# XiandaGuo/OpenStereo

Measured on NVIDIA H100. Metric: stereo_pairs_per_sec_gwcnet_256x512_d192, higher is better.
Workload: dtype f32

## Files before the change

openstereo_b200/csrc/conv3d_tcs2.cu:

```cuda
#include "tc_common.cuh"

namespace osb {

struct Tcs2Params {
  const float* x;
  const void* w;
  const float* scale;
  const float* shift;
  const float* residual;
  float* y;
  int B, D, H, Cin;
  int act;
  float kappa;
  unsigned int* overflow;
  int out_ndhwc, res_ndhwc;
  int items, hblocks;
  int Wr, ctiles;
  int ystride;
};

template <int COUT, int KC, int W, int TILES, bool GW = false>
struct Tcs2Cfg {
  static_assert(!GW || W == 128, "general-width tiles are 128-column segments of one output row");
  static constexpr int HALO = GW ? 1 : 0;
  static constexpr int CSTEP = 128 - HALO;
  static constexpr int R = 128 / W;
  static constexpr int ROWB = KC * 4;
  static constexpr int UNIT_BYTES = 128 * ROWB;
  static constexpr int N3 = 3 * COUT;
  static constexpr int G = 32;
  static constexpr int NG = COUT / G;
  static constexpr int B_SLICE = N3 * ROWB;
  static constexpr int B_SUB = 3 * G * ROWB;
  static constexpr int LD = 3 * G + 4;
  static constexpr int NLW = 5;
  static constexpr int FIXED_SMEM = 1024 + TC_BSLOTS * 3 * B_SUB + 128 * LD * 4 + 1024 + 2 * 4 * 2 * 32 * 4 + 3 * COUT * 4;
  static constexpr int STAGES = (232448 - FIXED_SMEM) / UNIT_BYTES < 10 ? (232448 - FIXED_SMEM) / UNIT_BYTES : 10;
  static_assert(STAGES >= NLW, "the ring must hold at least one unit per loader warp");
  static constexpr int NU = TILES * 3 * 2;
  static constexpr int HBLK = TILES * R;
  static constexpr int KSTEPS = KC / 16;
  static constexpr int LO = KC / 8;
  static constexpr int A_OFF = 0;
  static constexpr int B_OFF = A_OFF + STAGES * UNIT_BYTES;
  static constexpr int STAGE_OFF = B_OFF + TC_BSLOTS * 3 * B_SUB;
  static constexpr int BAR_OFF = STAGE_OFF + 128 * LD * 4;
  static constexpr int THREADS = 128 + 128 + 64;
  static constexpr size_t SMEM = 1024 + (size_t)BAR_OFF + 1024 + 2 * 4 * 2 * 32 * 4 + 3 * COUT * 4;
  static_assert(SMEM <= 232448, "shared memory budget of one CTA exceeded");
  static_assert(TILES == 1, "the consumer warpgroup holds one accumulator tile");
  static_assert(COUT % G == 0, "output channels come in groups of 32");
  static_assert(B_SUB % 1024 == 0 && UNIT_BYTES % 1024 == 0, "operand tiles must stay 1024-byte aligned");
};

template <int COUT, int KC, int W, int TILES, bool GW = false>
__global__ void __launch_bounds__(Tcs2Cfg<COUT, KC, W, TILES, GW>::THREADS, 1) conv3d_tcs2_kernel(const Tcs2Params p) {
  using C = Tcs2Cfg<COUT, KC, W, TILES, GW>;
  extern __shared__ __align__(1024) uint8_t smem_raw[];
  uint8_t* smem = reinterpret_cast<uint8_t*>((reinterpret_cast<uintptr_t>(smem_raw) + 1023) & ~static_cast<uintptr_t>(1023));
  uint8_t* a_buf = smem + C::A_OFF;
  uint8_t* b_buf = smem + C::B_OFF;
  float* stage = reinterpret_cast<float*>(smem + C::STAGE_OFF);
  uint64_t* bars = reinterpret_cast<uint64_t*>(smem + C::BAR_OFF);
  uint64_t* a_ready = bars;
  uint64_t* a_empty = a_ready + C::STAGES;
  uint64_t* b_full = a_empty + C::STAGES;
  uint64_t* b_empty = b_full + TC_BSLOTS * 3;
  float* xchg = reinterpret_cast<float*>(smem + C::BAR_OFF + 1024);
  float* s_scale = xchg + 2 * 4 * 2 * 32;
  float* s_shift = s_scale + COUT;
  float* zeros = s_shift + COUT;

  const int warp = threadIdx.x >> 5, lane = threadIdx.x & 31;
  const int nchunk = p.Cin / KC;
  const int Wp = GW ? p.Wr : W;
  const int YS = (W < 32 && p.ystride) ? p.ystride : COUT;
  const int ctiles = GW ? p.ctiles : 1;

  if (threadIdx.x == 0) {
    for (int s = 0; s < C::STAGES; ++s) {
      mbar_init(&a_ready[s], 32);
      mbar_init(&a_empty[s], 4);
    }
    for (int k = 0; k < TC_BSLOTS * 3; ++k) {
      mbar_init(&b_full[k], 1);
      mbar_init(&b_empty[k], 4);
    }
    fence_mbar_init();
  }
  for (int c = threadIdx.x; c < COUT; c += blockDim.x) {
    s_scale[c] = p.scale ? p.scale[c] : 1.f;
    s_shift[c] = p.shift ? p.shift[c] : 0.f;
    zeros[c] = 0.f;
  }
  __syncthreads();

  if (warp < 4) {
    const uint64_t dbase = (KC == 32) ? desc_sw128_base() : desc_sw64_base();
    constexpr uint32_t A_HALF = 64 * C::ROWB / 16;
    const uint32_t b16 = (smem_u32(b_buf) & 0x3FFFF) >> 4;
    const int Do = p.D / 2, Ho = p.H / 2;
    const int q = warp;
    const int m = q * 32 + lane;
    const int rr = m / W, wcol = m % W;
    const bool has_left_q = ((q * 32) % W) != 0;
    uint32_t unitc = 0, phc = 0, exc = 0;
    for (int it = blockIdx.x; it < p.items; it += gridDim.x) {
      const int cg = (it % C::NG) * C::G;
      const int it0 = it / C::NG;
      const int ct = it0 % ctiles;
      const int hb = (it0 / ctiles) % p.hblocks;
      const int d = (it0 / (ctiles * p.hblocks)) % Do;
      const int b = it0 / (ctiles * p.hblocks * Do);
      {
        float acc_e[2][C::G / 2], acc_o[2][C::G];
        uint32_t accum_e = 0, accum_o = 0;
        for (int kd = 0; kd < 3; ++kd) {
          const int din = 2 * d + kd - 1;
          if (din < 0 || din >= p.D) continue;
          for (int ch = 0; ch < nchunk; ++ch, ++phc) {
#pragma unroll
            for (int kh = 0; kh < 3; ++kh) {
              const uint32_t bslot = (phc & 1) * 3 + kh;
#pragma unroll
              for (int par = 0; par < 2; ++par) {
                const uint32_t slot = unitc % C::STAGES, ph = (unitc / C::STAGES) & 1;
                mbar_wait(&a_ready[slot], ph);
                if (par == 0) mbar_wait(&b_full[bslot], (phc >> 1) & 1);
                const uint64_t da0 = dbase | (uint64_t)((smem_u32(a_buf + slot * C::UNIT_BYTES) & 0x3FFFF) >> 4);
                const uint64_t db0 = dbase | (uint64_t)(b16 + (bslot * C::B_SUB + (par ? C::G * C::ROWB : 0)) / 16);
                wg_fence();
#pragma unroll
                for (int ks = 0; ks < C::KSTEPS; ++ks) {
                  if (par == 0) wg_mma_split<C::G>(acc_e, da0 + 2 * ks, A_HALF, db0 + 2 * ks, C::LO, ks > 0 ? 1u : accum_e);
                  else wg_mma_split<2 * C::G>(acc_o, da0 + 2 * ks, A_HALF, db0 + 2 * ks, C::LO, ks > 0 ? 1u : accum_o);
                }
                wg_commit();
                wg_wait_all();
                if (par == 0) accum_e = 1;
                else accum_o = 1;
                wg_release(&a_empty[slot], lane);
                if (par == 1) wg_release(&b_empty[bslot], lane);
                ++unitc;
              }
            }
          }
        }
        named_bar_sync(2, 128);
        wg_stage<C::G>(stage, C::LD, acc_e, warp, lane);
        wg_stage<2 * C::G>(stage + C::G, C::LD, acc_o, warp, lane);
        named_bar_sync(2, 128);
      }
      const int h0 = hb * C::HBLK;
      const int ntiles = min(TILES, (Ho - h0 + C::R - 1) / C::R);
      const int col = GW ? ct * C::CSTEP - C::HALO + m : wcol;
      const bool cvalid = !GW || (m >= C::HALO && col < Wp);
      const uint32_t vmask = GW ? __ballot_sync(0xffffffffu, cvalid) : 0xffffffffu;
      const float corr = 1.f + p.kappa * (float)(((d > 0) + 1 + (2 * d + 1 < p.D)) * nchunk * 3 * C::KSTEPS * 3);
      for (int t = 0; t < ntiles; ++t) {
        const int h = h0 + t * C::R + rr;
        const bool live = h < Ho;
        const ptrdiff_t vox = (((ptrdiff_t)b * Do + d) * Ho + h) * Wp + col;
        const size_t plane = (size_t)Do * Ho * Wp;
        const ptrdiff_t ncdhw0 = (ptrdiff_t)b * COUT * plane + ((ptrdiff_t)d * Ho + h) * Wp + col;
        {
          uint32_t raw[3][32];
#pragma unroll
          for (int kw = 0; kw < 3; ++kw)
#pragma unroll
            for (int c0 = 0; c0 < 32; c0 += 16) stage_ld16(stage + m * C::LD + kw * C::G + c0, &raw[kw][c0]);
          float* xb = xchg + (exc & 1) * (4 * 2 * 32);
          ++exc;
          if (lane == 31) {
#pragma unroll
            for (int i = 0; i < 32; ++i) xb[(q * 2) * 32 + i] = __uint_as_float(raw[1][i]);
          }
          named_bar_sync(1, 128);
          const float* xl = has_left_q ? xb + ((q - 1) * 2) * 32 : zeros;
          float out[32];
#pragma unroll
          for (int i0 = 0; i0 < 32; i0 += 4) {
            const float4 l4 = *reinterpret_cast<const float4*>(xl + i0);
            const float le[4] = {l4.x, l4.y, l4.z, l4.w};
#pragma unroll
            for (int k = 0; k < 4; ++k) {
              const int i = i0 + k;
              float left = __shfl_up_sync(0xffffffffu, __uint_as_float(raw[1][i]), 1);
              left = (lane == 0) ? le[k] : left;
              if (W < 32) left = (wcol == 0) ? 0.f : left;
              out[i] = ((left + __uint_as_float(raw[0][i])) + __uint_as_float(raw[2][i])) * corr;
            }
          }
          const uint32_t vm = (W < 32) ? __ballot_sync(0xffffffffu, live) : (live ? vmask : 0u);
          if (vm && p.out_ndhwc && (!p.residual || p.res_ndhwc)) {
            store_ndhwc_chunk32(stage + q * 32 * C::LD, lane, out, p.y + (vox - lane) * YS + cg,
                                p.residual ? p.residual + (vox - lane) * YS + cg : nullptr, YS, s_scale + cg, s_shift + cg, p.act,
                                vm);
          } else if (live && cvalid) {
#pragma unroll
            for (int i = 0; i < 32; ++i) out[i] = fmaf(out[i], s_scale[cg + i], s_shift[cg + i]);
            if (p.residual) {
              if (p.res_ndhwc) {
                const float4* rp = reinterpret_cast<const float4*>(p.residual + vox * YS + cg);
#pragma unroll
                for (int i = 0; i < 8; ++i) {
                  const float4 rv = __ldg(rp + i);
                  out[4 * i] += rv.x, out[4 * i + 1] += rv.y, out[4 * i + 2] += rv.z, out[4 * i + 3] += rv.w;
                }
              } else {
#pragma unroll
                for (int i = 0; i < 32; ++i) out[i] += __ldg(p.residual + ncdhw0 + (size_t)(cg + i) * plane);
              }
            }
            if (p.act == OSB_ACT_RELU) {
#pragma unroll
              for (int i = 0; i < 32; ++i) out[i] = fmaxf(out[i], 0.f);
            } else if (p.act == OSB_ACT_LEAKY) {
#pragma unroll
              for (int i = 0; i < 32; ++i) out[i] = out[i] > 0.f ? out[i] : 0.01f * out[i];
            }
            if (p.out_ndhwc) {
              float4* yp = reinterpret_cast<float4*>(p.y + vox * YS + cg);
#pragma unroll
              for (int i = 0; i < 8; ++i) yp[i] = make_float4(out[4 * i], out[4 * i + 1], out[4 * i + 2], out[4 * i + 3]);
            } else {
#pragma unroll
              for (int i = 0; i < 32; ++i) p.y[ncdhw0 + (size_t)(cg + i) * plane] = out[i];
            }
          }
        }
      }
    }
  }
  else if (warp < 8 || warp == 9) {
    const int lw = warp < 8 ? warp - 4 : 4;
    static_assert(KC == 16, "lane_voxel / unit-row mapping below is written for 64-byte operand rows");
    constexpr int CPR = KC / 4;
    constexpr int VPL = 32 / CPR;
    constexpr int NLD = 128 / VPL;
    static_assert(W % VPL == 0, "a load instruction must not straddle image rows");
    const int v0 = lane_voxel<KC>(lane), c = lane % CPR;
    float amax = 0.f;
    const int WI = 2 * Wp;
    const int Do = p.D / 2;
    uint32_t ubase = 0;
    int first = lw;
    auto fill = [&](const float* base, size_t rstride, size_t cstride, int h_first, int h_step, uint32_t u, int col0) {
      float4 v[NLD];
#pragma unroll
      for (int j = 0; j < NLD; ++j) {
        const int hin = h_first + h_step * ((VPL * j) / W);
        const size_t off = (size_t)((VPL * j) / W) * rstride + (size_t)((VPL * j) % W) * cstride;
        bool ok = hin >= 0 && hin < p.H;
        if (GW) ok = ok && (unsigned)(col0 + VPL * j) < (unsigned)Wp;
        v[j] = ok ? __ldg(reinterpret_cast<const float4*>(base + (ptrdiff_t)off)) : make_float4(0.f, 0.f, 0.f, 0.f);
      }
      const uint32_t slot = u % C::STAGES, ph = (u / C::STAGES) & 1;
      mbar_wait_relaxed(&a_empty[slot], ph ^ 1);
      uint8_t* tile = a_buf + slot * C::UNIT_BYTES;
#pragma unroll
      for (int j = 0; j < NLD; ++j) stage_f16_split<KC>(tile, v0 + VPL * j, c, v[j], amax);
      fence_proxy_async();
      mbar_arrive(&a_ready[slot]);
    };
    for (int it = blockIdx.x; it < p.items; it += gridDim.x) {
      const int it0 = it / C::NG;
      const int ct = it0 % ctiles;
      const int hb = (it0 / ctiles) % p.hblocks;
      const int od = (it0 / (ctiles * p.hblocks)) % Do;
      const int b = it0 / (ctiles * p.hblocks * Do);
      const int h0 = hb * C::HBLK;
      const int col0 = ct * C::CSTEP - C::HALO + v0;
      for (int kd = 0; kd < 3; ++kd) {
        const int din = 2 * od + kd - 1;
        if (din < 0 || din >= p.D) continue;
        const float* plane = p.x + ((size_t)b * p.D + din) * p.H * (size_t)WI * p.Cin;
        for (int ch = 0; ch < nchunk; ++ch) {
#pragma unroll 1
          for (int j = first; j < C::NU; j += C::NLW) {
            const int t = j / 6, kh = (j >> 1) % 3, par = j & 1;
            const int h_first = 2 * (h0 + t * C::R) + kh - 1;
            const float* base = plane + ((ptrdiff_t)h_first * WI + 2 * col0 + par) * p.Cin + ch * KC + c * 4;
            fill(base, (size_t)2 * WI * p.Cin, (size_t)2 * p.Cin, h_first, 2, ubase + j, col0);
          }
          ubase += C::NU;
          first = (first + C::NLW - C::NU % C::NLW) % C::NLW;
        }
      }
    }
    tc_report_overflow(p.overflow, amax);
  }
  else if (warp == 8) {
    if (elect_one()) {
      const uint8_t* wsrc = reinterpret_cast<const uint8_t*>(p.w);
      uint32_t phc = 0;
      for (int it = blockIdx.x; it < p.items; it += gridDim.x) {
        const int cg = (it % C::NG) * C::G;
        const int od = (it / C::NG / (ctiles * p.hblocks)) % (p.D / 2);
        for (int kd = 0; kd < 3; ++kd) {
          const int din = 2 * od + kd - 1;
          if (din < 0 || din >= p.D) continue;
          for (int ch = 0; ch < nchunk; ++ch, ++phc) {
            for (int kh = 0; kh < 3; ++kh) {
              const uint32_t slot = (phc & 1) * 3 + kh;
              const size_t slice = ((size_t)kd * nchunk + ch) * 3 + kh;
              mbar_wait_relaxed(&b_empty[slot], ((phc >> 1) & 1) ^ 1);
              mbar_arrive_expect_tx(&b_full[slot], C::B_SUB);
#pragma unroll
              for (int kw = 0; kw < 3; ++kw)
                bulk_g2s(b_buf + slot * C::B_SUB + kw * C::G * C::ROWB, wsrc + slice * C::B_SLICE + (size_t)(kw * COUT + cg) * C::ROWB,
                         C::G * C::ROWB, &b_full[slot]);
            }
          }
        }
      }
    }
    __syncwarp();
  }
}

template <int COUT, int KC, int W, int TILES, bool GW = false>
static int launch_tcs2(Tcs2Params& p, cudaStream_t stream) {
  using C = Tcs2Cfg<COUT, KC, W, TILES, GW>;
  auto kernel = conv3d_tcs2_kernel<COUT, KC, W, TILES, GW>;
  static PerDeviceFlag configured;
  if (!configured.here()) {
    cudaError_t e = cudaFuncSetAttribute(kernel, cudaFuncAttributeMaxDynamicSharedMemorySize, (int)C::SMEM);
    if (e != cudaSuccess) {
      set_error("conv3d_tcg: cannot reserve %zu bytes of shared memory: %s", C::SMEM, cudaGetErrorString(e));
      return OSB_ECUDA;
    }
    configured.here() = true;
  }
  if (W >= 32 && p.ystride && p.ystride != COUT) {
    set_error("conv3d_tcs2: channel slices are instantiated for W = 16 only");
    return OSB_EUNSUPPORTED;
  }
  p.hblocks = (p.H / 2 + C::HBLK - 1) / C::HBLK;
  if (GW) p.ctiles = (p.Wr + C::CSTEP - 1) / C::CSTEP;
  else p.Wr = W, p.ctiles = 1;
  const long long items = (long long)p.B * (p.D / 2) * p.hblocks * p.ctiles * C::NG;
  OSB_REQUIRE(items < (1ll << 31), "conv3d_tcs2: too many work items");
  p.items = (int)items;
  const int sms = sm_count();
  const int grid = (int)cap_persistent_grid(p.items < sms ? p.items : sms);
  static const std::string variant = tc_variant_name("tcs2<%d,%d,%d,%d,%d>", COUT, KC, W, TILES, (int)GW);
  set_tc_variant(variant.c_str());
  kernel<<<grid, C::THREADS, C::SMEM, stream>>>(p);
  count_launch();
  cudaError_t le = cudaGetLastError();
  if (le != cudaSuccess) {
    cudaFuncAttributes fa{};
    (void)cudaFuncGetAttributes(&fa, kernel);
    set_error("conv3d_tcs2_kernel<%d,%d,%d,%d>: launch failed: %s (threads %d, kernel maxThreadsPerBlock %d, regs %d, static smem %zu, "
              "dynamic smem %zu, max dynamic %d)", COUT, KC, W, TILES, cudaGetErrorString(le), C::THREADS, fa.maxThreadsPerBlock,
              fa.numRegs, fa.sharedSizeBytes, C::SMEM, fa.maxDynamicSharedSizeBytes);
    return OSB_ECUDA;
  }
  return OSB_OK;
}

}

extern "C" {

int osb_conv3d_s2_tc_supported(int Cin, int Cout, int D, int H, int W) {
  if (Cin % 16 != 0 || Cin < 16 || D % 2 || H % 2 || W % 2) return 0;
  if ((W == 128 && Cout == 64) || (W == 64 && (Cout == 64 || Cout == 96 || Cout == 128)) || (W == 32 && (Cout == 64 || Cout == 96)))
    return 1;
  return (osb_tc_general_width(W / 2) && (Cout == 64 || Cout == 128)) ? 1 : 0;
}

static int conv3d_k3_s2_tc_impl(const float* x_ndhwc, const void* w_split, const float* scale, const float* shift,
                                const float* residual, float* y, int B, int Cin, int Cout, int D, int H, int W, int act,
                                int out_ndhwc, int res_ndhwc, int ystride, osb_stream_t stream) {
  using namespace osb;
  OSB_REQUIRE(ystride == 0 || (ystride >= Cout && ystride % 4 == 0 && out_ndhwc && (!residual || res_ndhwc)),
              "conv3d_k3_s2_tc: a channel slice (ystride %d) needs channels-last tensors", ystride);
  OSB_REQUIRE(x_ndhwc && w_split && y, "conv3d_k3_s2_tc: null pointer");
  OSB_REQUIRE(B > 0 && D > 0 && H > 0, "conv3d_k3_s2_tc: empty shape");
  OSB_REQUIRE(osb_conv3d_s2_tc_supported(Cin, Cout, D, H, W), "conv3d_k3_s2_tc: unsupported shape Cin=%d Cout=%d D=%d H=%d W=%d", Cin,
              Cout, D, H, W);
  OSB_REQUIRE(act >= 0 && act <= 2, "conv3d_k3_s2_tc: unknown activation %d", act);
  Tcs2Params p{};
  p.x = x_ndhwc, p.w = w_split, p.scale = scale, p.shift = shift, p.residual = residual, p.y = y;
  p.B = B, p.D = D, p.H = H, p.Cin = Cin, p.act = act, p.out_ndhwc = out_ndhwc, p.res_ndhwc = res_ndhwc;
  p.kappa = rz_kappa(), p.overflow = tc_overflow_flag();
  p.ystride = ystride;
  OSB_REQUIRE(p.overflow, "tensor-core conv: cannot allocate the overflow flag");
  cudaStream_t s = (cudaStream_t)stream;
  if (W == 32 && Cout == 96) return launch_tcs2<96, 16, 16, 1>(p, s);
  if (W == 32 && Cout == 64) return launch_tcs2<64, 16, 16, 1>(p, s);
  if (W == 128 && Cout == 64) return launch_tcs2<64, 16, 64, 1>(p, s);
  if (W == 64 && Cout == 64) return launch_tcs2<64, 16, 32, 1>(p, s);
  if (W == 64 && Cout == 128) return launch_tcs2<128, 16, 32, 1>(p, s);
  if (W == 64 && Cout == 96) return launch_tcs2<96, 16, 32, 1>(p, s);
  p.Wr = W / 2;
  if (Cout == 64) return launch_tcs2<64, 16, 128, 1, true>(p, s);
  return launch_tcs2<128, 16, 128, 1, true>(p, s);
}

int osb_conv3d_k3_s2_tc_fwd(const float* x_ndhwc, const void* w_split, const float* scale, const float* shift,
                            const float* residual, float* y, int B, int Cin, int Cout, int D, int H, int W, int act,
                            int out_ndhwc, int res_ndhwc, osb_stream_t stream) {
  return conv3d_k3_s2_tc_impl(x_ndhwc, w_split, scale, shift, residual, y, B, Cin, Cout, D, H, W, act, out_ndhwc, res_ndhwc, 0, stream);
}

int osb_conv3d_k3_s2_tc_cs_fwd(const float* x_ndhwc, const void* w_split, const float* scale, const float* shift, float* y, int B,
                               int Cin, int Cout, int D, int H, int W, int act, int ystride, osb_stream_t stream) {
  return conv3d_k3_s2_tc_impl(x_ndhwc, w_split, scale, shift, nullptr, y, B, Cin, Cout, D, H, W, act, 1, 1, ystride, stream);
}
}
```

Measured before the change: 196.3.

## Share loaded input tiles across multiple consumer warpgroups in stride-2 conv3d

Lets several consumer warpgroups (TC_WGS) consume the same A-operand ring unit, each computing a different 32-channel output group, so the input tile is loaded once per item for several channel groups instead of once per group. The weight producer loads one B sub-tile per group into a wider slot, and warp registers are rebalanced with setmaxnreg. The epilogue stages accumulators in two 16-channel passes to fit per-warpgroup staging buffers. In exchange, shared memory per stage grows, fewer ring stages may fit, and warpgroups with no group to compute still have to wait and arrive on the barriers.

```diff
diff --git a/openstereo_b200/csrc/conv3d_tcs2.cu b/openstereo_b200/csrc/conv3d_tcs2.cu
--- a/openstereo_b200/csrc/conv3d_tcs2.cu
+++ b/openstereo_b200/csrc/conv3d_tcs2.cu
@@ -30,11 +30,16 @@
   static constexpr int N3 = 3 * COUT;
   static constexpr int G = 32;
   static constexpr int NG = COUT / G;
+  static constexpr int NP = (NG + TC_WGS - 1) / TC_WGS;
   static constexpr int B_SLICE = N3 * ROWB;
   static constexpr int B_SUB = 3 * G * ROWB;
-  static constexpr int LD = 3 * G + 4;
-  static constexpr int NLW = 5;
-  static constexpr int FIXED_SMEM = 1024 + TC_BSLOTS * 3 * B_SUB + 128 * LD * 4 + 1024 + 2 * 4 * 2 * 32 * 4 + 3 * COUT * 4;
+  static constexpr int B_SLOT = TC_WGS * B_SUB;
+  static constexpr int PC = 16;
+  static constexpr int NPASS = G / PC;
+  static constexpr int LD = 3 * PC + 4;
+  static constexpr int XCHG_FLOATS = 2 * 4 * PC;
+  static constexpr int NLW = 4;
+  static constexpr int FIXED_SMEM = 1024 + TC_BSLOTS * 3 * B_SLOT + TC_WGS * 128 * LD * 4 + 1024 + TC_WGS * XCHG_FLOATS * 4 + 3 * COUT * 4;
   static constexpr int STAGES = (232448 - FIXED_SMEM) / UNIT_BYTES < 10 ? (232448 - FIXED_SMEM) / UNIT_BYTES : 10;
   static_assert(STAGES >= NLW, "the ring must hold at least one unit per loader warp");
   static constexpr int NU = TILES * 3 * 2;
@@ -43,21 +48,36 @@
   static constexpr int LO = KC / 8;
   static constexpr int A_OFF = 0;
   static constexpr int B_OFF = A_OFF + STAGES * UNIT_BYTES;
-  static constexpr int STAGE_OFF = B_OFF + TC_BSLOTS * 3 * B_SUB;
-  static constexpr int BAR_OFF = STAGE_OFF + 128 * LD * 4;
-  static constexpr int THREADS = 128 + 128 + 64;
-  static constexpr size_t SMEM = 1024 + (size_t)BAR_OFF + 1024 + 2 * 4 * 2 * 32 * 4 + 3 * COUT * 4;
+  static constexpr int STAGE_OFF = B_OFF + TC_BSLOTS * 3 * B_SLOT;
+  static constexpr int BAR_OFF = STAGE_OFF + TC_WGS * 128 * LD * 4;
+  static constexpr int THREADS = TC_WG_THREADS;
+  static constexpr size_t SMEM = 1024 + (size_t)BAR_OFF + 1024 + TC_WGS * XCHG_FLOATS * 4 + 3 * COUT * 4;
   static_assert(SMEM <= 232448, "shared memory budget of one CTA exceeded");
-  static_assert(TILES == 1, "the consumer warpgroup holds one accumulator tile");
+  static_assert(TILES == 1, "a consumer warpgroup holds one accumulator tile");
   static_assert(COUT % G == 0, "output channels come in groups of 32");
+  static_assert(32 * LD >= TP_WARP_FLOATS, "store_ndhwc_chunk32 transposes through the warp's own rows of the staging tile");
   static_assert(B_SUB % 1024 == 0 && UNIT_BYTES % 1024 == 0, "operand tiles must stay 1024-byte aligned");
 };
+
+template <int N>
+__device__ __forceinline__ void s2_stage16(float* stage, int ld, const float (&acc)[2][N / 2], int c0, int dst, int wq, int lane) {
+#pragma unroll
+  for (int h = 0; h < 2; ++h) {
+    float* r0 = stage + (64 * h + 16 * wq + (lane >> 2)) * ld + 2 * (lane & 3) + dst;
+#pragma unroll
+    for (int jj = 0; jj < 2; ++jj) {
+      const int j = c0 / 8 + jj;
+      *reinterpret_cast<float2*>(r0 + 8 * jj) = make_float2(acc[h][4 * j], acc[h][4 * j + 1]);
+      *reinterpret_cast<float2*>(r0 + 8 * ld + 8 * jj) = make_float2(acc[h][4 * j + 2], acc[h][4 * j + 3]);
+    }
+  }
+}
 
 template <int COUT, int KC, int W, int TILES, bool GW = false>
 __global__ void __launch_bounds__(Tcs2Cfg<COUT, KC, W, TILES, GW>::THREADS, 1) conv3d_tcs2_kernel(const Tcs2Params p) {
   using C = Tcs2Cfg<COUT, KC, W, TILES, GW>;
   extern __shared__ __align__(1024) uint8_t smem_raw[];
-  uint8_t* smem = reinterpret_cast<uint8_t*>((reinterpret_cast<uintptr_t>(smem_raw) + 1023) & ~static_cast<uintptr_t>(1023));
+  uint8_t* smem = smem_raw + ((1024u - (smem_u32(smem_raw) & 1023u)) & 1023u);
   uint8_t* a_buf = smem + C::A_OFF;
   uint8_t* b_buf = smem + C::B_OFF;
   float* stage = reinterpret_cast<float*>(smem + C::STAGE_OFF);
@@ -67,7 +87,7 @@
   uint64_t* b_full = a_empty + C::STAGES;
   uint64_t* b_empty = b_full + TC_BSLOTS * 3;
   float* xchg = reinterpret_cast<float*>(smem + C::BAR_OFF + 1024);
-  float* s_scale = xchg + 2 * 4 * 2 * 32;
+  float* s_scale = xchg + TC_WGS * C::XCHG_FLOATS;
   float* s_shift = s_scale + COUT;
   float* zeros = s_shift + COUT;
 
@@ -80,11 +100,11 @@
   if (threadIdx.x == 0) {
     for (int s = 0; s < C::STAGES; ++s) {
       mbar_init(&a_ready[s], 32);
-      mbar_init(&a_empty[s], 4);
+      mbar_init(&a_empty[s], 4 * TC_WGS);
     }
     for (int k = 0; k < TC_BSLOTS * 3; ++k) {
       mbar_init(&b_full[k], 1);
-      mbar_init(&b_empty[k], 4);
+      mbar_init(&b_empty[k], 4 * TC_WGS);
     }
     fence_mbar_init();
   }
@@ -95,40 +115,47 @@
   }
   __syncthreads();
 
-  if (warp < 4) {
+  if (warp < 4 * TC_WGS) {
+    setmaxnreg_inc<TC_CONSUMER_REGS>();
+    const int wg = warp >> 2;
+    stage += wg * 128 * C::LD;
+    xchg += wg * C::XCHG_FLOATS;
+    const int bar_stage = 1 + 2 * wg, bar_xchg = 2 + 2 * wg;
     const uint64_t dbase = (KC == 32) ? desc_sw128_base() : desc_sw64_base();
     constexpr uint32_t A_HALF = 64 * C::ROWB / 16;
     const uint32_t b16 = (smem_u32(b_buf) & 0x3FFFF) >> 4;
     const int Do = p.D / 2, Ho = p.H / 2;
-    const int q = warp;
+    const int q = warp & 3;
     const int m = q * 32 + lane;
     const int rr = m / W, wcol = m % W;
     const bool has_left_q = ((q * 32) % W) != 0;
     uint32_t unitc = 0, phc = 0, exc = 0;
     for (int it = blockIdx.x; it < p.items; it += gridDim.x) {
-      const int cg = (it % C::NG) * C::G;
-      const int it0 = it / C::NG;
+      const int g = (it % C::NP) * TC_WGS + wg;
+      const bool has_group = g < C::NG;
+      const int cg = g * C::G;
+      const int it0 = it / C::NP;
       const int ct = it0 % ctiles;
       const int hb = (it0 / ctiles) % p.hblocks;
       const int d = (it0 / (ctiles * p.hblocks)) % Do;
       const int b = it0 / (ctiles * p.hblocks * Do);
-      {
-        float acc_e[2][C::G / 2], acc_o[2][C::G];
-        uint32_t accum_e = 0, accum_o = 0;
-        for (int kd = 0; kd < 3; ++kd) {
-          const int din = 2 * d + kd - 1;
-          if (din < 0 || din >= p.D) continue;
-          for (int ch = 0; ch < nchunk; ++ch, ++phc) {
-#pragma unroll
-            for (int kh = 0; kh < 3; ++kh) {
-              const uint32_t bslot = (phc & 1) * 3 + kh;
-#pragma unroll
-              for (int par = 0; par < 2; ++par) {
-                const uint32_t slot = unitc % C::STAGES, ph = (unitc / C::STAGES) & 1;
-                mbar_wait(&a_ready[slot], ph);
-                if (par == 0) mbar_wait(&b_full[bslot], (phc >> 1) & 1);
+      float acc_e[2][C::G / 2], acc_o[2][C::G];
+      uint32_t accum_e = 0, accum_o = 0;
+      for (int kd = 0; kd < 3; ++kd) {
+        const int din = 2 * d + kd - 1;
+        if (din < 0 || din >= p.D) continue;
+        for (int ch = 0; ch < nchunk; ++ch, ++phc) {
+#pragma unroll
+          for (int kh = 0; kh < 3; ++kh) {
+            const uint32_t bslot = (phc & 1) * 3 + kh;
+#pragma unroll
+            for (int par = 0; par < 2; ++par) {
+              const uint32_t slot = unitc % C::STAGES, ph = (unitc / C::STAGES) & 1;
+              mbar_wait(&a_ready[slot], ph);
+              if (par == 0) mbar_wait(&b_full[bslot], (phc >> 1) & 1);
+              if (has_group) {
                 const uint64_t da0 = dbase | (uint64_t)((smem_u32(a_buf + slot * C::UNIT_BYTES) & 0x3FFFF) >> 4);
-                const uint64_t db0 = dbase | (uint64_t)(b16 + (bslot * C::B_SUB + (par ? C::G * C::ROWB : 0)) / 16);
+                const uint64_t db0 = dbase | (uint64_t)(b16 + (bslot * C::B_SLOT + wg * C::B_SUB + (par ? C::G * C::ROWB : 0)) / 16);
                 wg_fence();
 #pragma unroll
                 for (int ks = 0; ks < C::KSTEPS; ++ks) {
@@ -139,101 +166,100 @@
                 wg_wait_all();
                 if (par == 0) accum_e = 1;
                 else accum_o = 1;
-                wg_release(&a_empty[slot], lane);
-                if (par == 1) wg_release(&b_empty[bslot], lane);
-                ++unitc;
               }
+              wg_release(&a_empty[slot], lane);
+              if (par == 1) wg_release(&b_empty[bslot], lane);
+              ++unitc;
             }
           }
         }
-        named_bar_sync(2, 128);
-        wg_stage<C::G>(stage, C::LD, acc_e, warp, lane);
-        wg_stage<2 * C::G>(stage + C::G, C::LD, acc_o, warp, lane);
-        named_bar_sync(2, 128);
-      }
-      const int h0 = hb * C::HBLK;
-      const int ntiles = min(TILES, (Ho - h0 + C::R - 1) / C::R);
+      }
+      if (!has_group) continue;
+      const int h = hb * C::HBLK + rr;
+      const bool live = h < Ho;
       const int col = GW ? ct * C::CSTEP - C::HALO + m : wcol;
       const bool cvalid = !GW || (m >= C::HALO && col < Wp);
       const uint32_t vmask = GW ? __ballot_sync(0xffffffffu, cvalid) : 0xffffffffu;
       const float corr = 1.f + p.kappa * (float)(((d > 0) + 1 + (2 * d + 1 < p.D)) * nchunk * 3 * C::KSTEPS * 3);
-      for (int t = 0; t < ntiles; ++t) {
-        const int h = h0 + t * C::R + rr;
-        const bool live = h < Ho;
-        const ptrdiff_t vox = (((ptrdiff_t)b * Do + d) * Ho + h) * Wp + col;
-        const size_t plane = (size_t)Do * Ho * Wp;
-        const ptrdiff_t ncdhw0 = (ptrdiff_t)b * COUT * plane + ((ptrdiff_t)d * Ho + h) * Wp + col;
-        {
-          uint32_t raw[3][32];
-#pragma unroll
-          for (int kw = 0; kw < 3; ++kw)
-#pragma unroll
-            for (int c0 = 0; c0 < 32; c0 += 16) stage_ld16(stage + m * C::LD + kw * C::G + c0, &raw[kw][c0]);
-          float* xb = xchg + (exc & 1) * (4 * 2 * 32);
-          ++exc;
-          if (lane == 31) {
-#pragma unroll
-            for (int i = 0; i < 32; ++i) xb[(q * 2) * 32 + i] = __uint_as_float(raw[1][i]);
+      const ptrdiff_t vox = (((ptrdiff_t)b * Do + d) * Ho + h) * Wp + col;
+      const size_t plane = (size_t)Do * Ho * Wp;
+      const ptrdiff_t ncdhw0 = (ptrdiff_t)b * COUT * plane + ((ptrdiff_t)d * Ho + h) * Wp + col;
+      float out[32];
+#pragma unroll
+      for (int pass = 0; pass < C::NPASS; ++pass) {
+        named_bar_sync(bar_stage, 128);
+        s2_stage16<C::G>(stage, C::LD, acc_e, pass * C::PC, 0, q, lane);
+        s2_stage16<2 * C::G>(stage, C::LD, acc_o, pass * C::PC, C::PC, q, lane);
+        s2_stage16<2 * C::G>(stage, C::LD, acc_o, C::G + pass * C::PC, 2 * C::PC, q, lane);
+        named_bar_sync(bar_stage, 128);
+        const float* srow = stage + m * C::LD;
+        float* xb = xchg + (exc & 1) * (4 * C::PC);
+        ++exc;
+        if (lane == 31) {
+#pragma unroll
+          for (int i = 0; i < C::PC; i += 4)
+            *reinterpret_cast<float4*>(xb + q * C::PC + i) = *reinterpret_cast<const float4*>(srow + C::PC + i);
+        }
+        named_bar_sync(bar_xchg, 128);
+        const float* xl = has_left_q ? xb + (q - 1) * C::PC : zeros;
+#pragma unroll
+        for (int i0 = 0; i0 < C::PC; i0 += 4) {
+          const float4 l4 = *reinterpret_cast<const float4*>(xl + i0);
+          const float4 p14 = *reinterpret_cast<const float4*>(srow + i0);
+          const float4 p04 = *reinterpret_cast<const float4*>(srow + C::PC + i0);
+          const float4 p24 = *reinterpret_cast<const float4*>(srow + 2 * C::PC + i0);
+          const float le[4] = {l4.x, l4.y, l4.z, l4.w};
+          const float p0[4] = {p04.x, p04.y, p04.z, p04.w}, p1[4] = {p14.x, p14.y, p14.z, p14.w}, p2[4] = {p24.x, p24.y, p24.z, p24.w};
+#pragma unroll
+          for (int k = 0; k < 4; ++k) {
+            float left = __shfl_up_sync(0xffffffffu, p0[k], 1);
+            left = (lane == 0) ? le[k] : left;
+            if (W < 32) left = (wcol == 0) ? 0.f : left;
+            out[pass * C::PC + i0 + k] = ((left + p1[k]) + p2[k]) * corr;
           }
-          named_bar_sync(1, 128);
-          const float* xl = has_left_q ? xb + ((q - 1) * 2) * 32 : zeros;
-          float out[32];
-#pragma unroll
-          for (int i0 = 0; i0 < 32; i0 += 4) {
-            const float4 l4 = *reinterpret_cast<const float4*>(xl + i0);
-            const float le[4] = {l4.x, l4.y, l4.z, l4.w};
-#pragma unroll
-            for (int k = 0; k < 4; ++k) {
-              const int i = i0 + k;
-              float left = __shfl_up_sync(0xffffffffu, __uint_as_float(raw[1][i]), 1);
-              left = (lane == 0) ? le[k] : left;
-              if (W < 32) left = (wcol == 0) ? 0.f : left;
-              out[i] = ((left + __uint_as_float(raw[0][i])) + __uint_as_float(raw[2][i])) * corr;
+        }
+      }
+      const uint32_t vm = (W < 32) ? __ballot_sync(0xffffffffu, live) : (live ? vmask : 0u);
+      if (vm && p.out_ndhwc && (!p.residual || p.res_ndhwc)) {
+        store_ndhwc_chunk32(stage + q * 32 * C::LD, lane, out, p.y + (vox - lane) * YS + cg,
+                            p.residual ? p.residual + (vox - lane) * YS + cg : nullptr, YS, s_scale + cg, s_shift + cg, p.act, vm);
+      } else if (live && cvalid) {
+#pragma unroll
+        for (int i = 0; i < 32; ++i) out[i] = fmaf(out[i], s_scale[cg + i], s_shift[cg + i]);
+        if (p.residual) {
+          if (p.res_ndhwc) {
+            const float4* rp = reinterpret_cast<const float4*>(p.residual + vox * YS + cg);
+#pragma unroll
+            for (int i = 0; i < 8; ++i) {
+              const float4 rv = __ldg(rp + i);
+              out[4 * i] += rv.x, out[4 * i + 1] += rv.y, out[4 * i + 2] += rv.z, out[4 * i + 3] += rv.w;
             }
+          } else {
+#pragma unroll
+            for (int i = 0; i < 32; ++i) out[i] += __ldg(p.residual + ncdhw0 + (size_t)(cg + i) * plane);
           }
-          const uint32_t vm = (W < 32) ? __ballot_sync(0xffffffffu, live) : (live ? vmask : 0u);
-          if (vm && p.out_ndhwc && (!p.residual || p.res_ndhwc)) {
-            store_ndhwc_chunk32(stage + q * 32 * C::LD, lane, out, p.y + (vox - lane) * YS + cg,
-                                p.residual ? p.residual + (vox - lane) * YS + cg : nullptr, YS, s_scale + cg, s_shift + cg, p.act,
-                                vm);
-          } else if (live && cvalid) {
-#pragma unroll
-            for (int i = 0; i < 32; ++i) out[i] = fmaf(out[i], s_scale[cg + i], s_shift[cg + i]);
-            if (p.residual) {
-              if (p.res_ndhwc) {
-                const float4* rp = reinterpret_cast<const float4*>(p.residual + vox * YS + cg);
-#pragma unroll
-                for (int i = 0; i < 8; ++i) {
-                  const float4 rv = __ldg(rp + i);
-                  out[4 * i] += rv.x, out[4 * i + 1] += rv.y, out[4 * i + 2] += rv.z, out[4 * i + 3] += rv.w;
-                }
-              } else {
-#pragma unroll
-                for (int i = 0; i < 32; ++i) out[i] += __ldg(p.residual + ncdhw0 + (size_t)(cg + i) * plane);
-              }
-            }
-            if (p.act == OSB_ACT_RELU) {
-#pragma unroll
-              for (int i = 0; i < 32; ++i) out[i] = fmaxf(out[i], 0.f);
-            } else if (p.act == OSB_ACT_LEAKY) {
-#pragma unroll
-              for (int i = 0; i < 32; ++i) out[i] = out[i] > 0.f ? out[i] : 0.01f * out[i];
-            }
-            if (p.out_ndhwc) {
-              float4* yp = reinterpret_cast<float4*>(p.y + vox * YS + cg);
-#pragma unroll
-              for (int i = 0; i < 8; ++i) yp[i] = make_float4(out[4 * i], out[4 * i + 1], out[4 * i + 2], out[4 * i + 3]);
-            } else {
-#pragma unroll
-              for (int i = 0; i < 32; ++i) p.y[ncdhw0 + (size_t)(cg + i) * plane] = out[i];
-            }
-          }
-        }
-      }
-    }
-  }
-  else if (warp < 8 || warp == 9) {
-    const int lw = warp < 8 ? warp - 4 : 4;
+        }
+        if (p.act == OSB_ACT_RELU) {
+#pragma unroll
+          for (int i = 0; i < 32; ++i) out[i] = fmaxf(out[i], 0.f);
+        } else if (p.act == OSB_ACT_LEAKY) {
+#pragma unroll
+          for (int i = 0; i < 32; ++i) out[i] = out[i] > 0.f ? out[i] : 0.01f * out[i];
+        }
+        if (p.out_ndhwc) {
+          float4* yp = reinterpret_cast<float4*>(p.y + vox * YS + cg);
+#pragma unroll
+          for (int i = 0; i < 8; ++i) yp[i] = make_float4(out[4 * i], out[4 * i + 1], out[4 * i + 2], out[4 * i + 3]);
+        } else {
+#pragma unroll
+          for (int i = 0; i < 32; ++i) p.y[ncdhw0 + (size_t)(cg + i) * plane] = out[i];
+        }
+      }
+    }
+  }
+  else if (warp < 4 * TC_WGS + C::NLW) {
+    setmaxnreg_dec<TC_LOADER_REGS>();
+    const int lw = warp - 4 * TC_WGS;
     static_assert(KC == 16, "lane_voxel / unit-row mapping below is written for 64-byte operand rows");
     constexpr int CPR = KC / 4;
     constexpr int VPL = 32 / CPR;
@@ -264,7 +290,7 @@
       mbar_arrive(&a_ready[slot]);
     };
     for (int it = blockIdx.x; it < p.items; it += gridDim.x) {
-      const int it0 = it / C::NG;
+      const int it0 = it / C::NP;
       const int ct = it0 % ctiles;
       const int hb = (it0 / ctiles) % p.hblocks;
       const int od = (it0 / (ctiles * p.hblocks)) % Do;
@@ -290,13 +316,15 @@
     }
     tc_report_overflow(p.overflow, amax);
   }
-  else if (warp == 8) {
-    if (elect_one()) {
+  else {
+    setmaxnreg_dec<TC_PRODUCER_REGS>();
+    if (warp == 4 * TC_WGS + C::NLW && elect_one()) {
       const uint8_t* wsrc = reinterpret_cast<const uint8_t*>(p.w);
       uint32_t phc = 0;
       for (int it = blockIdx.x; it < p.items; it += gridDim.x) {
-        const int cg = (it % C::NG) * C::G;
-        const int od = (it / C::NG / (ctiles * p.hblocks)) % (p.D / 2);
+        const int g0 = (it % C::NP) * TC_WGS;
+        const int ngr = min(TC_WGS, C::NG - g0);
+        const int od = (it / C::NP / (ctiles * p.hblocks)) % (p.D / 2);
         for (int kd = 0; kd < 3; ++kd) {
           const int din = 2 * od + kd - 1;
           if (din < 0 || din >= p.D) continue;
@@ -305,11 +333,12 @@
               const uint32_t slot = (phc & 1) * 3 + kh;
               const size_t slice = ((size_t)kd * nchunk + ch) * 3 + kh;
               mbar_wait_relaxed(&b_empty[slot], ((phc >> 1) & 1) ^ 1);
-              mbar_arrive_expect_tx(&b_full[slot], C::B_SUB);
-#pragma unroll
-              for (int kw = 0; kw < 3; ++kw)
-                bulk_g2s(b_buf + slot * C::B_SUB + kw * C::G * C::ROWB, wsrc + slice * C::B_SLICE + (size_t)(kw * COUT + cg) * C::ROWB,
-                         C::G * C::ROWB, &b_full[slot]);
+              mbar_arrive_expect_tx(&b_full[slot], ngr * C::B_SUB);
+              for (int t = 0; t < ngr; ++t)
+#pragma unroll
+                for (int kw = 0; kw < 3; ++kw)
+                  bulk_g2s(b_buf + slot * C::B_SLOT + t * C::B_SUB + kw * C::G * C::ROWB,
+                           wsrc + slice * C::B_SLICE + (size_t)(kw * COUT + (g0 + t) * C::G) * C::ROWB, C::G * C::ROWB, &b_full[slot]);
             }
           }
         }
@@ -339,7 +368,7 @@
   p.hblocks = (p.H / 2 + C::HBLK - 1) / C::HBLK;
   if (GW) p.ctiles = (p.Wr + C::CSTEP - 1) / C::CSTEP;
   else p.Wr = W, p.ctiles = 1;
-  const long long items = (long long)p.B * (p.D / 2) * p.hblocks * p.ctiles * C::NG;
+  const long long items = (long long)p.B * (p.D / 2) * p.hblocks * p.ctiles * C::NP;
   OSB_REQUIRE(items < (1ll << 31), "conv3d_tcs2: too many work items");
   p.items = (int)items;
   const int sms = sm_count();
```

New measurement: 202.8, median of 6. 3.3% higher.
